# WLBF/flex-gpu-scheduler

Measured on AMD Instinct MI355X. Metric: pods/sec sched throughput + p99 PodGroup gang-admit latency, 1/2/4/8-GPU groups, higher is better.
Workload: dtype int64

## Files before the change

csrc/common/json.cc:

```cpp
#include "common/json.h"

#include <cerrno>
#include <cmath>
#include <cstdio>
#include <cstring>

namespace xsched {

namespace {
const std::string kEmptyString;
const Json::Array kEmptyArray;
const Json::Object kEmptyObject;

class Parser {
 public:
  explicit Parser(std::string_view s) : p_(s.data()), end_(s.data() + s.size()) {}

  Json parse_document() {
    ws();
    Json v = value(0);
    ws();
    if (p_ != end_) fail("trailing characters");
    return v;
  }

  void parse_array_stream(const std::function<void(Json&&)>& fn) {
    ws();
    if (p_ >= end_ || *p_ != '[') fail("expected a JSON array");
    ++p_;
    ws();
    if (p_ < end_ && *p_ == ']') {
      ++p_;
    } else {
      for (;;) {
        ws();
        fn(value(1));
        ws();
        if (p_ < end_ && *p_ == ',') { ++p_; continue; }
        if (p_ < end_ && *p_ == ']') { ++p_; break; }
        fail("expected ',' or ']'");
      }
    }
    ws();
    if (p_ != end_) fail("trailing characters");
  }

 private:
  const char* p_;
  const char* end_;

  [[noreturn]] void fail(const char* what) {
    throw JsonError(std::string("json parse error: ") + what);
  }
  void ws() {
    while (p_ < end_ && (*p_ == ' ' || *p_ == '\n' || *p_ == '\r' || *p_ == '\t')) ++p_;
  }
  bool lit(const char* l, size_t n) {
    if (static_cast<size_t>(end_ - p_) >= n && std::memcmp(p_, l, n) == 0) {
      p_ += n;
      return true;
    }
    return false;
  }

  Json value(int depth) {
    if (depth > 256) fail("nesting too deep");
    if (p_ >= end_) fail("unexpected end");
    switch (*p_) {
      case '{': return object(depth);
      case '[': return array(depth);
      case '"': return Json(string());
      case 't': if (lit("true", 4)) return Json(true); fail("bad literal");
      case 'f': if (lit("false", 5)) return Json(false); fail("bad literal");
      case 'n': if (lit("null", 4)) return Json(); fail("bad literal");
      default: return number();
    }
  }

  Json object(int depth) {
    ++p_;
    Json o = Json::object();
    auto& m = o.members_mut();
    ws();
    if (p_ < end_ && *p_ == '}') { ++p_; return o; }
    for (;;) {
      ws();
      if (p_ >= end_ || *p_ != '"') fail("expected key");
      std::string k = string();
      ws();
      if (p_ >= end_ || *p_ != ':') fail("expected ':'");
      ++p_;
      ws();
      Json v = value(depth + 1);
      bool replaced = false;
      for (auto& kv : m) {
        if (kv.first == k) { kv.second = std::move(v); replaced = true; break; }
      }
      if (!replaced) m.emplace_back(std::move(k), std::move(v));
      ws();
      if (p_ < end_ && *p_ == ',') { ++p_; continue; }
      if (p_ < end_ && *p_ == '}') { ++p_; return o; }
      fail("expected ',' or '}'");
    }
  }

  Json array(int depth) {
    ++p_;
    Json a = Json::array();
    auto& items = a.items_mut();
    ws();
    if (p_ < end_ && *p_ == ']') { ++p_; return a; }
    for (;;) {
      ws();
      items.push_back(value(depth + 1));
      ws();
      if (p_ < end_ && *p_ == ',') { ++p_; continue; }
      if (p_ < end_ && *p_ == ']') { ++p_; return a; }
      fail("expected ',' or ']'");
    }
  }

  static void put_utf8(std::string& out, uint32_t cp) {
    if (cp < 0x80) {
      out.push_back(static_cast<char>(cp));
    } else if (cp < 0x800) {
      out.push_back(static_cast<char>(0xC0 | (cp >> 6)));
      out.push_back(static_cast<char>(0x80 | (cp & 0x3F)));
    } else if (cp < 0x10000) {
      out.push_back(static_cast<char>(0xE0 | (cp >> 12)));
      out.push_back(static_cast<char>(0x80 | ((cp >> 6) & 0x3F)));
      out.push_back(static_cast<char>(0x80 | (cp & 0x3F)));
    } else {
      out.push_back(static_cast<char>(0xF0 | (cp >> 18)));
      out.push_back(static_cast<char>(0x80 | ((cp >> 12) & 0x3F)));
      out.push_back(static_cast<char>(0x80 | ((cp >> 6) & 0x3F)));
      out.push_back(static_cast<char>(0x80 | (cp & 0x3F)));
    }
  }

  uint32_t hex4() {
    if (end_ - p_ < 4) fail("bad \\u escape");
    uint32_t v = 0;
    for (int i = 0; i < 4; ++i) {
      char c = *p_++;
      v <<= 4;
      if (c >= '0' && c <= '9') v |= c - '0';
      else if (c >= 'a' && c <= 'f') v |= c - 'a' + 10;
      else if (c >= 'A' && c <= 'F') v |= c - 'A' + 10;
      else fail("bad hex digit");
    }
    return v;
  }

  std::string string() {
    ++p_;
    std::string out;
    const char* run = p_;
    while (p_ < end_) {
      char c = *p_;
      if (c == '"') {
        out.append(run, p_);
        ++p_;
        return out;
      }
      if (c == '\\') {
        out.append(run, p_);
        ++p_;
        if (p_ >= end_) fail("bad escape");
        char e = *p_++;
        switch (e) {
          case '"': out.push_back('"'); break;
          case '\\': out.push_back('\\'); break;
          case '/': out.push_back('/'); break;
          case 'b': out.push_back('\b'); break;
          case 'f': out.push_back('\f'); break;
          case 'n': out.push_back('\n'); break;
          case 'r': out.push_back('\r'); break;
          case 't': out.push_back('\t'); break;
          case 'u': {
            uint32_t cp = hex4();
            if (cp >= 0xD800 && cp <= 0xDBFF && end_ - p_ >= 6 && p_[0] == '\\' && p_[1] == 'u') {
              p_ += 2;
              uint32_t lo = hex4();
              cp = 0x10000 + ((cp - 0xD800) << 10) + (lo - 0xDC00);
            }
            put_utf8(out, cp);
            break;
          }
          default: fail("bad escape");
        }
        run = p_;
        continue;
      }
      ++p_;
    }
    fail("unterminated string");
  }

  Json number() {
    const char* start = p_;
    bool is_float = false;
    if (p_ < end_ && (*p_ == '-' || *p_ == '+')) ++p_;
    while (p_ < end_) {
      char c = *p_;
      if (c >= '0' && c <= '9') { ++p_; continue; }
      if (c == '.' || c == 'e' || c == 'E' || c == '-' || c == '+') { is_float = true; ++p_; continue; }
      break;
    }
    if (p_ == start) fail("unexpected character");
    std::string tok(start, p_);
    if (!is_float) {
      errno = 0;
      char* e = nullptr;
      long long v = std::strtoll(tok.c_str(), &e, 10);
      if (errno == 0 && e && *e == '\0') return Json(static_cast<int64_t>(v));
    }
    char* e = nullptr;
    double d = std::strtod(tok.c_str(), &e);
    if (!e || *e != '\0') fail("bad number");
    return Json(d);
  }
};

void dump_string(std::string& out, const std::string& s) {
  out.push_back('"');
  for (unsigned char c : s) {
    switch (c) {
      case '"': out += "\\\""; break;
      case '\\': out += "\\\\"; break;
      case '\n': out += "\\n"; break;
      case '\r': out += "\\r"; break;
      case '\t': out += "\\t"; break;
      case '\b': out += "\\b"; break;
      case '\f': out += "\\f"; break;
      default:
        if (c < 0x20) {
          char buf[8];
          std::snprintf(buf, sizeof buf, "\\u%04x", c);
          out += buf;
        } else {
          out.push_back(static_cast<char>(c));
        }
    }
  }
  out.push_back('"');
}
}

const std::string& Json::as_string() const { return t_ == Type::String ? h_.s : kEmptyString; }
const Json::Array& Json::items() const { return t_ == Type::Array ? h_.a : kEmptyArray; }
Json::Array& Json::items_mut() {
  if (t_ != Type::Array) { *this = array(); }
  return h_.a;
}
const Json::Object& Json::members() const { return t_ == Type::Object ? h_.o : kEmptyObject; }
Json::Object& Json::members_mut() {
  if (t_ != Type::Object) { *this = object(); }
  return h_.o;
}

const Json* Json::get(std::string_view key) const {
  if (t_ != Type::Object) return nullptr;
  for (const auto& kv : h_.o)
    if (kv.first == key) return &kv.second;
  return nullptr;
}

Json* Json::get_mut(std::string_view key) {
  if (t_ != Type::Object) return nullptr;
  for (auto& kv : h_.o)
    if (kv.first == key) return &kv.second;
  return nullptr;
}

const Json* Json::path(std::initializer_list<std::string_view> keys) const {
  const Json* cur = this;
  for (auto k : keys) {
    cur = cur->get(k);
    if (!cur) return nullptr;
  }
  return cur;
}

const Json& Json::operator[](std::string_view key) const {
  const Json* v = get(key);
  return v ? *v : json_null();
}

Json& Json::set(std::string_view key, Json v) {
  auto& m = members_mut();
  for (auto& kv : m) {
    if (kv.first == key) {
      kv.second = std::move(v);
      return kv.second;
    }
  }
  m.emplace_back(std::string(key), std::move(v));
  return m.back().second;
}

Json& Json::at_or_create(std::string_view key) {
  auto& m = members_mut();
  for (auto& kv : m)
    if (kv.first == key) {
      if (!kv.second.is_object()) kv.second = object();
      return kv.second;
    }
  m.emplace_back(std::string(key), object());
  return m.back().second;
}

bool Json::erase(std::string_view key) {
  if (t_ != Type::Object) return false;
  for (auto it = h_.o.begin(); it != h_.o.end(); ++it) {
    if (it->first == key) {
      h_.o.erase(it);
      return true;
    }
  }
  return false;
}

void Json::push_back(Json v) { items_mut().push_back(std::move(v)); }

bool Json::operator==(const Json& o) const {
  if (is_number() && o.is_number()) {
    if (t_ == Type::Int && o.t_ == Type::Int) return i_ == o.i_;
    return as_double() == o.as_double();
  }
  if (t_ != o.t_) return false;
  switch (t_) {
    case Type::Null: return true;
    case Type::Bool: return i_ == o.i_;
    case Type::String: return h_.s == o.h_.s;
    case Type::Array: return h_.a == o.h_.a;
    case Type::Object: {
      if (h_.o.size() != o.h_.o.size()) return false;
      for (const auto& kv : h_.o) {
        const Json* other = o.get(kv.first);
        if (!other || !(*other == kv.second)) return false;
      }
      return true;
    }
    default: return false;
  }
}

void Json::dump_to(std::string& out) const {
  switch (t_) {
    case Type::Null: out += "null"; break;
    case Type::Bool: out += i_ ? "true" : "false"; break;
    case Type::Int: out += std::to_string(i_); break;
    case Type::Double: {
      if (!std::isfinite(d_)) { out += "null"; break; }
      char buf[32];
      std::snprintf(buf, sizeof buf, "%.17g", d_);
      out += buf;
      break;
    }
    case Type::String: dump_string(out, h_.s); break;
    case Type::Array: {
      out.push_back('[');
      bool first = true;
      for (const auto& v : h_.a) {
        if (!first) out.push_back(',');
        first = false;
        v.dump_to(out);
      }
      out.push_back(']');
      break;
    }
    case Type::Object: {
      out.push_back('{');
      bool first = true;
      for (const auto& kv : h_.o) {
        if (!first) out.push_back(',');
        first = false;
        dump_string(out, kv.first);
        out.push_back(':');
        kv.second.dump_to(out);
      }
      out.push_back('}');
      break;
    }
  }
}

std::string Json::dump() const {
  std::string out;
  out.reserve(256);
  dump_to(out);
  return out;
}

Json Json::parse(std::string_view text) { return Parser(text).parse_document(); }

void Json::parse_array_stream(std::string_view text, const std::function<void(Json&&)>& fn) {
  Parser(text).parse_array_stream(fn);
}

void Json::merge_patch(const Json& patch) {
  if (!patch.is_object()) {
    *this = patch;
    return;
  }
  if (!is_object()) *this = object();
  for (const auto& kv : patch.h_.o) {
    if (kv.second.is_null()) {
      erase(kv.first);
    } else if (kv.second.is_object()) {
      Json* cur = get_mut(kv.first);
      if (cur && cur->is_object()) {
        cur->merge_patch(kv.second);
      } else {
        Json fresh = object();
        fresh.merge_patch(kv.second);
        set(kv.first, std::move(fresh));
      }
    } else {
      set(kv.first, kv.second);
    }
  }
}

Json Json::diff_merge_patch(const Json& from, const Json& to) {
  if (!from.is_object() || !to.is_object()) return to;
  Json patch = object();
  for (const auto& kv : from.h_.o) {
    if (!to.get(kv.first)) patch.set(kv.first, Json());
  }
  for (const auto& kv : to.h_.o) {
    const Json* old = from.get(kv.first);
    if (!old) {
      patch.set(kv.first, kv.second);
    } else if (!(*old == kv.second)) {
      if (old->is_object() && kv.second.is_object())
        patch.set(kv.first, diff_merge_patch(*old, kv.second));
      else
        patch.set(kv.first, kv.second);
    }
  }
  return patch;
}

namespace {
inline uint64_t mix(uint64_t h, uint64_t v) {
  h ^= v;
  h *= 0xff51afd7ed558ccdULL;
  return h ^ (h >> 33);
}
inline uint64_t fnv(uint64_t h, const void* data, size_t n) {
  const unsigned char* p = static_cast<const unsigned char*>(data);
  h = mix(h, n);
  for (; n >= 8; n -= 8, p += 8) {
    uint64_t w;
    std::memcpy(&w, p, 8);
    h = mix(h, w);
  }
  if (n) {
    uint64_t w = 0;
    std::memcpy(&w, p, n);
    h = mix(h, w);
  }
  return h;
}
}

uint64_t json_hash(const Json& j, uint64_t h, std::string_view skip_key) {
  uint8_t tag = static_cast<uint8_t>(j.type());
  h = fnv(h, &tag, 1);
  switch (j.type()) {
    case Json::Type::Null:
      break;
    case Json::Type::Bool: {
      uint8_t b = j.as_bool() ? 1 : 0;
      h = fnv(h, &b, 1);
      break;
    }
    case Json::Type::Int: {
      int64_t v = j.as_int();
      h = fnv(h, &v, sizeof v);
      break;
    }
    case Json::Type::Double: {
      double v = j.as_double();
      h = fnv(h, &v, sizeof v);
      break;
    }
    case Json::Type::String:
      h = fnv(h, j.as_string().data(), j.as_string().size());
      break;
    case Json::Type::Array:
      for (const auto& x : j.items()) h = json_hash(x, h);
      break;
    case Json::Type::Object:
      for (const auto& [k, v] : j.members()) {
        if (!skip_key.empty() && k == skip_key) continue;
        h = fnv(h, k.data(), k.size());
        h = json_hash(v, h);
      }
      break;
  }
  return h;
}

}
```

csrc/store/store.cc:

```cpp
#include "store/store.h"

#include "common/clock.h"

#include <algorithm>
#include <chrono>
#include <cstdio>
#include <thread>

#include "api/types.h"

namespace xsched {

const char* event_type_name(EventType t) {
  switch (t) {
    case EventType::Added: return "ADDED";
    case EventType::Modified: return "MODIFIED";
    case EventType::Deleted: return "DELETED";
    case EventType::Bookmark: return "BOOKMARK";
  }
  return "UNKNOWN";
}

void Watcher::push(const WatchEvent& ev) {
  {
    std::lock_guard<AdaptiveMutex> g(mu_);
    q_.push_back(ev);
  }
  cv_.notify_one();
}

void Watcher::push_batch(std::vector<WatchEvent> evs) {
  {
    std::lock_guard<AdaptiveMutex> g(mu_);
    for (auto& e : evs) q_.push_back(std::move(e));
  }
  cv_.notify_one();
}

bool Watcher::push_quiet(const WatchEvent& ev) {
  std::lock_guard<AdaptiveMutex> g(mu_);
  q_.push_back(ev);
  return waiters_ > 0;
}

bool Watcher::push_batch_quiet(std::vector<WatchEvent> evs) {
  std::lock_guard<AdaptiveMutex> g(mu_);
  for (auto& e : evs) q_.push_back(std::move(e));
  return waiters_ > 0;
}

std::vector<WatchEvent> Watcher::next(int timeout_ms, size_t max) {
  std::vector<WatchEvent> out;
  std::unique_lock<AdaptiveMutex> lk(mu_);
  if (q_.empty() && !stopped_.load()) {
    ++waiters_;
    if (timeout_ms < 0)
      cv_.wait(lk, [&] { return !q_.empty() || stopped_.load(); });
    else
      cv_.wait_for(lk, std::chrono::milliseconds(timeout_ms), [&] { return !q_.empty() || stopped_.load(); });
    --waiters_;
  }
  size_t n = std::min(max, q_.size());
  out.reserve(n);
  for (size_t i = 0; i < n; ++i) {
    out.push_back(std::move(q_.front()));
    q_.pop_front();
  }
  return out;
}

void Watcher::stop() {
  {
    std::lock_guard<AdaptiveMutex> g(mu_);
    stopped_.store(true);
  }
  cv_.notify_all();
}

size_t Watcher::pending() const {
  std::lock_guard<AdaptiveMutex> g(mu_);
  return q_.size();
}

ObjectStore::~ObjectStore() {
  {
    std::lock_guard<std::mutex> g(reap_mu_);
    reap_stop_ = true;
  }
  reap_cv_.notify_all();
  if (reaper_.joinable()) reaper_.join();
}

void ObjectStore::reap(std::vector<WatchEvent>&& dead) const {
  {
    std::lock_guard<std::mutex> g(reap_mu_);
    if (reap_stop_) return;
    if (!reaper_.joinable()) reaper_ = std::thread([this] { reaper_loop(); });
    if (reap_q_.empty()) {
      reap_q_.swap(dead);
    } else {
      for (auto& e : dead) reap_q_.push_back(std::move(e));
    }
  }
  reap_cv_.notify_one();
}

void ObjectStore::reaper_loop() const {
  name_this_thread("xs-reaper");
  std::unique_lock<std::mutex> lk(reap_mu_);
  for (;;) {
    reap_cv_.wait(lk, [&] { return reap_stop_ || !reap_q_.empty(); });
    std::vector<WatchEvent> batch;
    batch.swap(reap_q_);
    lk.unlock();
    batch.clear();
    lk.lock();
    if (reap_stop_ && reap_q_.empty()) return;
  }
}

ObjectStore::ObjectStore() {
  uid_salt_ = static_cast<uint64_t>(std::chrono::steady_clock::now().time_since_epoch().count());
}

bool ObjectStore::namespaced(const std::string& kind) {
  return !(kind == "nodes" || kind == "priorityclasses" || kind == "noderesourcetopologies" || kind == "namespaces" ||
           kind == "loadwatchermetrics" || kind == "persistentvolumes" || kind == "storageclasses" ||
           kind == "csinodes");
}

void ObjectStore::stamp(Json& obj, int64_t rv) {
  obj.at_or_create("metadata").set("resourceVersion", Json(std::to_string(rv)));
}

void ObjectStore::check_faults(const std::string& verb, const std::string& kind) {
  if (!has_faults_.load(std::memory_order_relaxed)) return;
  int delay = 0;
  bool fail = false;
  {
    std::lock_guard<std::mutex> g(fault_mu_);
    for (auto& r : faults_) {
      if (r.remaining == 0) continue;
      if ((r.verb == "*" || r.verb == verb) && (r.kind == "*" || r.kind == kind)) {
        if (r.remaining > 0) --r.remaining;
        delay += r.delay_us;
        if (r.fail_prob > 0.0 && std::uniform_real_distribution<double>(0, 1)(fault_rng_) < r.fail_prob) fail = true;
      }
    }
  }
  if (delay > 0) std::this_thread::sleep_for(std::chrono::microseconds(delay));
  if (fail) throw StoreError(500, "InternalError", "injected fault: " + verb + " " + kind);
}

void ObjectStore::add_fault(const FaultRule& r) {
  std::lock_guard<std::mutex> g(fault_mu_);
  faults_.push_back(r);
  has_faults_.store(true);
}

void ObjectStore::clear_faults() {
  std::lock_guard<std::mutex> g(fault_mu_);
  faults_.clear();
  has_faults_.store(false);
}

void ObjectStore::emit_locked(EventType t, const std::string& kind, const JsonPtr& obj, const JsonPtr& old, int64_t rv,
                              bool status_only) {
  WatchEvent ev{t, kind, obj, old, rv, status_only};
  if (batch_) {
    batch_->push_back(ev);
  } else {
    const Json& md = (*obj)["metadata"];
    const std::string& ns = md["namespace"].as_string();
    for (auto& w : watchers_)
      if (!w->stopped() && w->wants(kind, ns) && w->push_quiet(ev) &&
          std::find(wake_.begin(), wake_.end(), w) == wake_.end())
        wake_.push_back(w);
  }
  history_.push_back(std::move(ev));
  if (history_.size() > history_cap_) {
    compacted_rv_ = history_.front().rv;
    evicted_.push_back(std::move(history_.front()));
    history_.pop_front();
  }
}

JsonPtr ObjectStore::create_locked(const std::string& kind, Json obj) {
  Json& md = obj.at_or_create("metadata");
  std::string name = md["name"].as_string();
  if (name.empty()) {
    std::string gen = md["generateName"].as_string();
    if (gen.empty()) throw StoreError(422, "Invalid", "metadata.name: Required value");
    char buf[16];
    std::snprintf(buf, sizeof buf, "%05llx", static_cast<unsigned long long>((uid_counter_ * 2654435761u) & 0xfffff));
    name = gen + buf;
    md.set("name", Json(name));
  }
  std::string ns = md["namespace"].as_string();
  if (namespaced(kind) && ns.empty()) {
    ns = "default";
    md.set("namespace", Json(ns));
  }
  auto& km = kinds_[kind];
  std::string key = key_of(namespaced(kind) ? ns : "", name);
  if (km.count(key)) throw StoreError(409, "AlreadyExists", kind + " \"" + name + "\" already exists");
  ++uid_counter_;
  char uid[48];
  uint64_t a = uid_counter_ ^ uid_salt_;
  std::snprintf(uid, sizeof uid, "%08llx-%04llx-4%03llx-8%03llx-%012llx",
                static_cast<unsigned long long>(a & 0xffffffff), static_cast<unsigned long long>((a >> 32) & 0xffff),
                static_cast<unsigned long long>((a >> 48) & 0xfff), static_cast<unsigned long long>(uid_counter_ & 0xfff),
                static_cast<unsigned long long>(uid_counter_));
  if (md["uid"].as_string().empty()) md.set("uid", Json(std::string(uid)));
  if (!md["creationTimestamp"].is_string()) md.set("creationTimestamp", Json(format_rfc3339(wall_now_us())));
  if (kind == "pods") {
    Json& st = obj.at_or_create("status");
    if (!st["phase"].is_string()) st.set("phase", Json("Pending"));
  }
  int64_t rv = rv_.fetch_add(1) + 1;
  stamp(obj, rv);
  auto ptr = std::make_shared<const Json>(std::move(obj));
  km[key] = Entry{ptr};
  emit_locked(EventType::Added, kind, ptr, nullptr, rv);
  if (kind == "events") expire_events_locked(key);
  return ptr;
}

void ObjectStore::set_event_ttl_us(int64_t ttl_us) {
  Guard g(*this);
  event_ttl_us_ = ttl_us;
}

void ObjectStore::expire_events_locked(const std::string& created_key) {
  const int64_t now = wall_now_us();
  event_expiry_.emplace_back(now, created_key);
  auto& km = kinds_["events"];
  while (!event_expiry_.empty() && now - event_expiry_.front().first >= event_ttl_us_) {
    auto it = km.find(event_expiry_.front().second);
    event_expiry_.pop_front();
    if (it == km.end()) continue;
    JsonPtr old = it->second.obj;
    km.erase(it);
    emit_locked(EventType::Deleted, "events", old, old, rv_.fetch_add(1) + 1);
  }
}

JsonPtr ObjectStore::create(const std::string& kind, Json obj) {
  check_faults("create", kind);
  Guard g(*this);
  return create_locked(kind, std::move(obj));
}

std::vector<JsonPtr> ObjectStore::create_many(const std::string& kind, std::vector<Json> objs) {
  check_faults("create", kind);
  std::vector<JsonPtr> out;
  out.reserve(objs.size());
  Guard g(*this);
  std::vector<WatchEvent> batch;
  batch_ = &batch;
  try {
    for (auto& o : objs) out.push_back(create_locked(kind, std::move(o)));
  } catch (...) {
    batch_ = nullptr;
    flush_batch_locked(batch);
    throw;
  }
  batch_ = nullptr;
  flush_batch_locked(batch);
  return out;
}

size_t ObjectStore::create_chunked(const std::string& kind,
                                  const std::function<void(const std::function<void(Json&&)>&)>& produce) {
  auto group_of = [](const Json& o) -> const std::string& {
    return o["metadata"]["labels"]["pod-group.scheduling.sigs.k8s.io"].as_string();
  };
  std::vector<Json> chunk;
  chunk.reserve(2 * kCreateChunk);
  size_t n = 0;
  auto flush = [&] {
    if (chunk.empty()) return;
    n += create_many(kind, std::move(chunk)).size();
    chunk.clear();
  };
  produce([&](Json&& o) {
    if (chunk.size() >= kCreateChunk) {
      const std::string& g = group_of(o);
      if (g.empty() || g != group_of(chunk.back())) flush();
    }
    chunk.push_back(std::move(o));
  });
  flush();
  return n;
}

void ObjectStore::flush_batch_locked(std::vector<WatchEvent>& batch) {
  for (auto& w : watchers_) {
    if (w->stopped()) continue;
    std::vector<WatchEvent> mine;
    mine.reserve(batch.size());
    for (const auto& ev : batch) {
      const std::string& ns = (*ev.obj)["metadata"]["namespace"].as_string();
      if (w->wants(ev.kind, ns)) mine.push_back(ev);
    }
    if (!mine.empty() && w->push_batch_quiet(std::move(mine)) && std::find(wake_.begin(), wake_.end(), w) == wake_.end())
      wake_.push_back(w);
  }
}

JsonPtr ObjectStore::get(const std::string& kind, const std::string& ns, const std::string& name) const {
  Guard g(*this);
  auto kit = kinds_.find(kind);
  if (kit == kinds_.end()) return nullptr;
  auto it = kit->second.find(key_of(namespaced(kind) ? ns : "", name));
  return it == kit->second.end() ? nullptr : it->second.obj;
}

std::vector<JsonPtr> ObjectStore::list(const std::string& kind, const std::string& ns, int64_t* rv_out) const {
  std::vector<JsonPtr> out;
  Guard g(*this);
  if (rv_out) *rv_out = rv_.load();
  auto kit = kinds_.find(kind);
  if (kit == kinds_.end()) return out;
  out.reserve(kit->second.size());
  for (const auto& kv : kit->second) {
    if (!ns.empty() && (*kv.second.obj)["metadata"]["namespace"].as_string() != ns) continue;
    out.push_back(kv.second.obj);
  }
  return out;
}

size_t ObjectStore::count(const std::string& kind) const {
  Guard g(*this);
  auto kit = kinds_.find(kind);
  return kit == kinds_.end() ? 0 : kit->second.size();
}

JsonPtr ObjectStore::update(const std::string& kind, Json obj, bool check_rv) {
  check_faults("update", kind);
  Guard g(*this);
  const Json& md = obj["metadata"];
  std::string ns = namespaced(kind) ? md["namespace"].str_or("default") : "";
  std::string name = md["name"].as_string();
  auto& km = kinds_[kind];
  auto it = km.find(key_of(ns, name));
  if (it == km.end()) throw StoreError(404, "NotFound", kind + " \"" + name + "\" not found");
  const Json& cur_md = (*it->second.obj)["metadata"];
  if (check_rv && md["resourceVersion"].is_string() &&
      md["resourceVersion"].as_string() != cur_md["resourceVersion"].as_string())
    throw StoreError(409, "Conflict",
                     "Operation cannot be fulfilled on " + kind + " \"" + name +
                         "\": the object has been modified; please apply your changes to the latest version and try again");
  Json& nmd = obj.at_or_create("metadata");
  nmd.set("uid", cur_md["uid"]);
  nmd.set("creationTimestamp", cur_md["creationTimestamp"]);
  if (ns.size()) nmd.set("namespace", Json(ns));
  int64_t rv = rv_.fetch_add(1) + 1;
  stamp(obj, rv);
  auto ptr = std::make_shared<const Json>(std::move(obj));
  JsonPtr old = it->second.obj;
  it->second.obj = ptr;
  emit_locked(EventType::Modified, kind, ptr, old, rv);
  return ptr;
}

JsonPtr ObjectStore::update_optimistic(const std::string& kind, const std::string& key, const std::string& name,
                                       const std::function<std::optional<Json>(const Json& cur)>& build,
                                       bool status_only) {
  for (;;) {
    JsonPtr base;
    {
      Guard g(*this);
      auto& km = kinds_[kind];
      auto it = km.find(key);
      if (it == km.end()) throw StoreError(404, "NotFound", kind + " \"" + name + "\" not found");
      base = it->second.obj;
    }
    std::optional<Json> next = build(*base);
    Guard g(*this);
    auto& km = kinds_[kind];
    auto it = km.find(key);
    if (it == km.end()) throw StoreError(404, "NotFound", kind + " \"" + name + "\" not found");
    if (it->second.obj != base) continue;
    if (!next) return base;
    int64_t rv = rv_.fetch_add(1) + 1;
    stamp(*next, rv);
    auto ptr = std::make_shared<const Json>(std::move(*next));
    it->second.obj = ptr;
    emit_locked(EventType::Modified, kind, ptr, base, rv, status_only);
    return ptr;
  }
}

JsonPtr ObjectStore::patch(const std::string& kind, const std::string& ns, const std::string& name,
                           const Json& merge_patch) {
  check_faults("patch", kind);
  bool status_only = merge_patch.is_object() && merge_patch.size() > 0;
  for (const auto& [k, v] : merge_patch.members()) {
    if (k == "status") continue;
    if (k == "metadata" && v.is_object() && v.size() == 1 && v.get("resourceVersion")) continue;
    status_only = false;
  }
  return update_optimistic(kind, key_of(namespaced(kind) ? ns : "", name), name,
                           [&](const Json& cur) -> std::optional<Json> {
    if (const Json* pmd = merge_patch.get("metadata")) {
      const Json& prv = (*pmd)["resourceVersion"];
      if (prv.is_string() && !prv.as_string().empty() && prv.as_string() != cur["metadata"]["resourceVersion"].as_string())
        throw StoreError(409, "Conflict",
                         "Operation cannot be fulfilled on " + kind + " \"" + name +
                             "\": the object has been modified; please apply your changes to the latest version and try again");
    }
    Json obj = cur;
    Json saved_md = obj["metadata"];
    obj.merge_patch(merge_patch);
    Json& md = obj.at_or_create("metadata");
    for (const char* k : {"uid", "creationTimestamp", "name", "namespace"})
      if (const Json* v = saved_md.get(k)) md.set(k, *v);
    if (obj == cur) return std::nullopt;
    return obj;
  }, status_only);
}

JsonPtr ObjectStore::remove(const std::string& kind, const std::string& ns, const std::string& name,
                            int64_t grace_seconds, const std::string& uid_precondition) {
  check_faults("delete", kind);
  Guard g(*this);
  auto& km = kinds_[kind];
  auto it = km.find(key_of(namespaced(kind) ? ns : "", name));
  if (it == km.end()) throw StoreError(404, "NotFound", kind + " \"" + name + "\" not found");
  if (!uid_precondition.empty() && (*it->second.obj)["metadata"]["uid"].as_string() != uid_precondition)
    throw StoreError(409, "Conflict", "Precondition failed: UID in precondition does not match");
  if (kind == "pods" && grace_seconds > 0) {
    Json obj = *it->second.obj;
    Json& md = obj.at_or_create("metadata");
    if (md["deletionTimestamp"].is_string()) return it->second.obj;
    md.set("deletionTimestamp", Json(format_rfc3339(wall_now_us() + grace_seconds * 1000000)));
    md.set("deletionGracePeriodSeconds", Json(grace_seconds));
    int64_t rv = rv_.fetch_add(1) + 1;
    stamp(obj, rv);
    auto ptr = std::make_shared<const Json>(std::move(obj));
    JsonPtr old = it->second.obj;
    it->second.obj = ptr;
    emit_locked(EventType::Modified, kind, ptr, old, rv);
    return ptr;
  }
  JsonPtr old = it->second.obj;
  km.erase(it);
  shrink_locked(km);
  int64_t rv = rv_.fetch_add(1) + 1;
  emit_locked(EventType::Deleted, kind, old, old, rv);
  return old;
}

void ObjectStore::shrink_locked(KindMap& km) {
  if (km.bucket_count() > 4096 && km.size() * 8 < km.bucket_count()) km.rehash(0);
}

size_t ObjectStore::remove_many(const std::string& kind, const std::string& ns,
                                const std::vector<std::string>& names) {
  check_faults("delete", kind);
  Guard g(*this);
  auto& km = kinds_[kind];
  std::vector<WatchEvent> batch;
  batch_ = &batch;
  size_t n = 0;
  for (const auto& name : names) {
    auto it = km.find(key_of(namespaced(kind) ? ns : "", name));
    if (it == km.end()) continue;
    JsonPtr old = it->second.obj;
    km.erase(it);
    int64_t rv = rv_.fetch_add(1) + 1;
    emit_locked(EventType::Deleted, kind, old, old, rv);
    ++n;
  }
  shrink_locked(km);
  batch_ = nullptr;
  flush_batch_locked(batch);
  return n;
}

size_t ObjectStore::delete_all(const std::string& kind, const std::string& ns) {
  Guard g(*this);
  auto kit = kinds_.find(kind);
  if (kit == kinds_.end()) return 0;
  size_t n = 0;
  std::vector<WatchEvent> batch;
  batch_ = &batch;
  struct Flush {
    ObjectStore* s;
    std::vector<WatchEvent>* b;
    ~Flush() {
      s->batch_ = nullptr;
      s->flush_batch_locked(*b);
    }
  } flush{this, &batch};
  for (auto it = kit->second.begin(); it != kit->second.end();) {
    if (!ns.empty() && (*it->second.obj)["metadata"]["namespace"].as_string() != ns) {
      ++it;
      continue;
    }
    JsonPtr old = it->second.obj;
    it = kit->second.erase(it);
    int64_t rv = rv_.fetch_add(1) + 1;
    emit_locked(EventType::Deleted, kind, old, old, rv);
    ++n;
    if (batch.size() >= kCreateChunk) {
      flush_batch_locked(batch);
      batch.clear();
    }
  }
  return n;
}

JsonPtr ObjectStore::bind(const std::string& ns, const std::string& name, const std::string& uid,
                          const std::string& node, const Json& annotations) {
  check_faults("bind", "pods");
  const std::string now = format_rfc3339(wall_now_us());
  return update_optimistic("pods", key_of(ns, name), name, [&](const Json& cur) -> std::optional<Json> {
    if (!uid.empty() && cur["metadata"]["uid"].as_string() != uid)
      throw StoreError(409, "Conflict", "Precondition failed: UID in precondition does not match");
    if (!cur["spec"]["nodeName"].as_string().empty())
      throw StoreError(409, "Conflict",
                       "pod " + name + " is already assigned to node \"" + cur["spec"]["nodeName"].as_string() + "\"");
    if (cur["metadata"]["deletionTimestamp"].is_string())
      throw StoreError(409, "Conflict", "pod " + name + " is being deleted, cannot be assigned to a host");
    Json obj = cur;
    obj.at_or_create("spec").set("nodeName", Json(node));
    if (annotations.is_object() && annotations.size()) {
      Json& ann = obj.at_or_create("metadata").at_or_create("annotations");
      for (const auto& kv : annotations.members()) ann.set(kv.first, kv.second);
    }
    Json& st = obj.at_or_create("status");
    Json cond = Json::object();
    cond.set("type", Json("PodScheduled"));
    cond.set("status", Json("True"));
    cond.set("lastTransitionTime", Json(now));
    Json conds = Json::array();
    for (const auto& c : st["conditions"].items())
      if (c["type"].as_string() != "PodScheduled") conds.push_back(c);
    conds.push_back(std::move(cond));
    st.set("conditions", std::move(conds));
    return obj;
  });
}

WatcherPtr ObjectStore::watch(const std::set<std::string>& kinds, const std::string& ns, int64_t since_rv) {
  auto w = std::make_shared<Watcher>(kinds, ns);
  Guard g(*this);
  if (since_rv > 0) {
    if (since_rv < compacted_rv_)
      throw StoreError(410, "Expired", "too old resource version: " + std::to_string(since_rv));
    for (const auto& ev : history_) {
      if (ev.rv <= since_rv) continue;
      const std::string& ens = (*ev.obj)["metadata"]["namespace"].as_string();
      if (w->wants(ev.kind, ens)) w->push(ev);
    }
  }
  watchers_.push_back(w);
  return w;
}

void ObjectStore::unwatch(const WatcherPtr& w) {
  w->stop();
  Guard g(*this);
  for (auto it = watchers_.begin(); it != watchers_.end(); ++it) {
    if (*it == w) {
      watchers_.erase(it);
      break;
    }
  }
}

}
```

csrc/store/store.h:

```cpp
#pragma once

#include "common/adaptive_mutex.h"

#include <atomic>
#include <condition_variable>
#include <cstdint>
#include <deque>
#include <functional>
#include <map>
#include <memory>
#include <mutex>
#include <optional>
#include <random>
#include <set>
#include <string>
#include <thread>
#include <unordered_map>
#include <vector>

#include "common/json.h"

namespace xsched {

class StoreError : public std::runtime_error {
 public:
  StoreError(int code, const std::string& reason, const std::string& msg)
      : std::runtime_error(msg), code_(code), reason_(reason) {}
  int code() const { return code_; }
  const std::string& reason() const { return reason_; }

 private:
  int code_;
  std::string reason_;
};

enum class EventType : uint8_t { Added, Modified, Deleted, Bookmark };
const char* event_type_name(EventType t);

struct WatchEvent {
  EventType type;
  std::string kind;
  JsonPtr obj;
  JsonPtr old;
  int64_t rv = 0;
  bool status_only = false;
};

class Watcher {
 public:
  explicit Watcher(std::set<std::string> kinds, std::string ns) : kinds_(std::move(kinds)), ns_(std::move(ns)) {}
  std::vector<WatchEvent> next(int timeout_ms, size_t max = 4096);
  void stop();
  bool stopped() const { return stopped_.load(); }
  size_t pending() const;
  bool wants(const std::string& kind, const std::string& ns) const {
    return (kinds_.empty() || kinds_.count(kind)) && (ns_.empty() || ns.empty() || ns == ns_);
  }
  void push(const WatchEvent& ev);
  void push_batch(std::vector<WatchEvent> evs);
  bool push_quiet(const WatchEvent& ev);
  bool push_batch_quiet(std::vector<WatchEvent> evs);
  void notify() { cv_.notify_one(); }

 private:
  std::set<std::string> kinds_;
  std::string ns_;
  mutable AdaptiveMutex mu_;
  std::condition_variable_any cv_;
  std::deque<WatchEvent> q_;
  int waiters_ = 0;
  std::atomic<bool> stopped_{false};
};
using WatcherPtr = std::shared_ptr<Watcher>;

struct FaultRule {
  std::string verb;
  std::string kind;
  double fail_prob = 0.0;
  int delay_us = 0;
  int remaining = -1;
};

class ObjectStore {
 public:
  ObjectStore();
  ~ObjectStore();

  JsonPtr create(const std::string& kind, Json obj);
  JsonPtr get(const std::string& kind, const std::string& ns, const std::string& name) const;
  std::vector<JsonPtr> list(const std::string& kind, const std::string& ns, int64_t* rv_out = nullptr) const;
  JsonPtr update(const std::string& kind, Json obj, bool check_rv = true);
  JsonPtr patch(const std::string& kind, const std::string& ns, const std::string& name, const Json& merge_patch);
  JsonPtr remove(const std::string& kind, const std::string& ns, const std::string& name, int64_t grace_seconds = 0,
                 const std::string& uid_precondition = "");
  JsonPtr bind(const std::string& ns, const std::string& name, const std::string& uid, const std::string& node,
               const Json& annotations);

  WatcherPtr watch(const std::set<std::string>& kinds, const std::string& ns = "", int64_t since_rv = 0);
  void unwatch(const WatcherPtr& w);

  int64_t resource_version() const { return rv_.load(); }
  size_t count(const std::string& kind) const;

  void add_fault(const FaultRule& r);
  void clear_faults();

  void set_event_ttl_us(int64_t ttl_us);

  std::vector<JsonPtr> create_many(const std::string& kind, std::vector<Json> objs);
  static constexpr size_t kCreateChunk = 64;
  size_t create_chunked(const std::string& kind,
                        const std::function<void(const std::function<void(Json&&)>&)>& produce);
  size_t delete_all(const std::string& kind, const std::string& ns = "");
  size_t remove_many(const std::string& kind, const std::string& ns, const std::vector<std::string>& names);

  static std::string key_of(const std::string& ns, const std::string& name) { return ns.empty() ? name : ns + "/" + name; }
  static bool namespaced(const std::string& kind);

 private:
  struct Entry {
    JsonPtr obj;
  };
  using KindMap = std::unordered_map<std::string, Entry>;

  void check_faults(const std::string& verb, const std::string& kind);
  void expire_events_locked(const std::string& created_key);
  void emit_locked(EventType t, const std::string& kind, const JsonPtr& obj, const JsonPtr& old, int64_t rv,
                   bool status_only = false);
  JsonPtr create_locked(const std::string& kind, Json obj);
  void flush_batch_locked(std::vector<WatchEvent>& batch);
  static void stamp(Json& obj, int64_t rv);
  JsonPtr update_optimistic(const std::string& kind, const std::string& key, const std::string& name,
                            const std::function<std::optional<Json>(const Json& cur)>& build, bool status_only = false);
  std::vector<WatchEvent>* batch_ = nullptr;

  mutable AdaptiveMutex mu_;
  class Guard {
   public:
    explicit Guard(const ObjectStore& s) : s_(s) { s_.mu_.lock(); }
    ~Guard() {
      std::vector<WatchEvent> dead;
      if (!s_.evicted_.empty()) dead.swap(s_.evicted_);
      std::vector<WatcherPtr> wake;
      if (!s_.wake_.empty()) wake.swap(s_.wake_);
      s_.mu_.unlock();
      for (const auto& w : wake) w->notify();
      if (!dead.empty()) s_.reap(std::move(dead));
    }
    Guard(const Guard&) = delete;
    Guard& operator=(const Guard&) = delete;

   private:
    const ObjectStore& s_;
  };
  mutable std::vector<WatchEvent> evicted_;
  mutable std::vector<WatcherPtr> wake_;
  void reap(std::vector<WatchEvent>&& dead) const;
  void reaper_loop() const;
  mutable std::mutex reap_mu_;
  mutable std::condition_variable reap_cv_;
  mutable std::vector<WatchEvent> reap_q_;
  mutable std::thread reaper_;
  mutable bool reap_stop_ = false;
  void shrink_locked(KindMap& km);
  std::unordered_map<std::string, KindMap> kinds_;
  std::atomic<int64_t> rv_{0};
  std::vector<WatcherPtr> watchers_;
  std::deque<WatchEvent> history_;
  size_t history_cap_ = 50000;
  int64_t event_ttl_us_ = 3600LL * 1000000;
  std::deque<std::pair<int64_t, std::string>> event_expiry_;
  int64_t compacted_rv_ = 0;
  uint64_t uid_counter_ = 0;
  uint64_t uid_salt_;

  std::mutex fault_mu_;
  std::vector<FaultRule> faults_;
  std::atomic<bool> has_faults_{false};
  std::mt19937_64 fault_rng_{12345};
};

}
```

flex_gpu_scheduler_amd/build_ext.py:

```python
from __future__ import annotations

import argparse
import concurrent.futures as cf
import os
import shutil
import subprocess
import sys
import sysconfig
from pathlib import Path

ROOT = Path(__file__).resolve().parent.parent
CSRC = ROOT / "csrc"
PKG = ROOT / "flex_gpu_scheduler_amd"
BUILD = ROOT / "build"
HIP_ARCH = os.environ.get("PYTORCH_ROCM_ARCH", "gfx950")
ROCM = Path(os.environ.get("ROCM_PATH", "/opt/rocm"))

CORE_DIRS = ["common", "api", "store", "framework", "scheduler", "plugins", "rest", "apiserver"]
LINK_LIBS = ["-lssl", "-lcrypto"]
CXXFLAGS = ["-std=c++20", "-O3", "-fPIC", "-Wall", "-Wno-unused-variable", "-Wno-unused-parameter",
            "-Wno-sign-compare", "-fvisibility=hidden", "-pthread",
            *os.environ.get("XSCHED_CXXFLAGS_EXTRA", "").split()]


def _ext_suffix() -> str:
    return sysconfig.get_config_var("EXT_SUFFIX") or ".so"


def core_sources() -> list[Path]:
    out = []
    for d in CORE_DIRS:
        out.extend(sorted((CSRC / d).glob("*.cc")))
    return out


def _headers_mtime() -> float:
    hs = list(CSRC.rglob("*.h"))
    return max((h.stat().st_mtime for h in hs), default=0.0)


def _jobs() -> int:
    env = os.environ.get("MAX_JOBS")
    if env and env.isdigit():
        return max(1, int(env))
    return max(1, min(16, os.cpu_count() or 4))


def _compile(cmd: list[str], src: Path) -> None:
    r = subprocess.run(cmd, capture_output=True, text=True)
    if r.returncode != 0:
        raise RuntimeError(f"compile failed for {src}:\n{' '.join(cmd)}\n{r.stderr[-8000:]}")


def build_objects(srcs: list[Path], objdir: Path, extra: list[str], includes: list[str]) -> list[Path]:
    objdir.mkdir(parents=True, exist_ok=True)
    hmt = _headers_mtime()
    todo = []
    objs = []
    for s in srcs:
        o = objdir / (s.relative_to(CSRC).as_posix().replace("/", "__") + ".o")
        objs.append(o)
        if o.exists() and o.stat().st_mtime >= max(s.stat().st_mtime, hmt):
            continue
        cmd = ["g++", *CXXFLAGS, *extra, *[f"-I{i}" for i in includes], "-c", str(s), "-o", str(o)]
        todo.append((cmd, s))
    if todo:
        with cf.ThreadPoolExecutor(_jobs()) as ex:
            futs = [ex.submit(_compile, c, s) for c, s in todo]
            for f in futs:
                f.result()
    return objs


def build_core(verbose: bool = True) -> Path:
    import pybind11

    py_inc = sysconfig.get_paths()["include"]
    includes = [str(CSRC), pybind11.get_include(), py_inc, str(ROCM / "include")]
    srcs = core_sources() + sorted((CSRC / "telemetry").glob("*.cc")) + [CSRC / "python" / "bindings.cc"]
    objs = build_objects(srcs, BUILD / "core", [], includes)
    out = PKG / f"_xsched{_ext_suffix()}"
    newest = max(o.stat().st_mtime for o in objs)
    if not out.exists() or out.stat().st_mtime < newest:
        cmd = ["g++", "-shared", "-pthread", *[str(o) for o in objs], *LINK_LIBS, "-o", str(out)]
        r = subprocess.run(cmd, capture_output=True, text=True)
        if r.returncode != 0:
            raise RuntimeError(f"link failed:\n{r.stderr[-8000:]}")
        if verbose:
            print(f"[build_ext] linked {out.relative_to(ROOT)}")
    return out


def build_core_debuginfo(verbose: bool = True) -> Path:
    import pybind11

    py_inc = sysconfig.get_paths()["include"]
    includes = [str(CSRC), pybind11.get_include(), py_inc, str(ROCM / "include")]
    srcs = core_sources() + sorted((CSRC / "telemetry").glob("*.cc")) + [CSRC / "python" / "bindings.cc"]
    objs = build_objects(srcs, BUILD / "core_g", ["-g1", "-gz"], includes)
    out = ROOT / "dbg" / f"_xsched{_ext_suffix()}"
    out.parent.mkdir(exist_ok=True)
    cmd = ["g++", "-shared", "-pthread", *[str(o) for o in objs], *LINK_LIBS, "-o", str(out)]
    r = subprocess.run(cmd, capture_output=True, text=True)
    if r.returncode != 0:
        raise RuntimeError(f"link failed:\n{r.stderr[-8000:]}")
    if verbose:
        print(f"[build_ext] linked {out.relative_to(ROOT)}")
    return out


def build_hip(verbose: bool = True) -> Path | None:
    hipcc = shutil.which("hipcc") or str(ROCM / "bin" / "hipcc")
    if not Path(hipcc).exists():
        raise RuntimeError("hipcc not found; the HIP probes require ROCm")
    srcs = sorted((CSRC / "hip").glob("*.hip"))
    if not srcs:
        return None
    out = PKG / "ops" / "_hipprobe.so"
    newest = max([s.stat().st_mtime for s in srcs] + [_headers_mtime()])
    if out.exists() and out.stat().st_mtime >= newest:
        return out
    cmd = [hipcc, f"--offload-arch={HIP_ARCH}", "-O3", "-std=c++17", "-fPIC", "-shared",
           f"-I{CSRC}", *[str(s) for s in srcs], "-o", str(out)]
    r = subprocess.run(cmd, capture_output=True, text=True)
    if r.returncode != 0:
        raise RuntimeError(f"hipcc failed:\n{' '.join(cmd)}\n{r.stderr[-8000:]}")
    if verbose:
        print(f"[build_ext] built {out.relative_to(ROOT)} for {HIP_ARCH}")
    return out


def build_stream_sweep(verbose: bool = True) -> Path:
    hipcc = shutil.which("hipcc") or str(ROCM / "bin" / "hipcc")
    src = CSRC / "tools" / "stream_sweep.hip"
    out = PKG / "ops" / "stream_sweep"
    if out.exists() and out.stat().st_mtime >= src.stat().st_mtime:
        return out
    cmd = [hipcc, f"--offload-arch={HIP_ARCH}", "-O3", "-std=c++17", str(src), "-o", str(out)]
    r = subprocess.run(cmd, capture_output=True, text=True)
    if r.returncode != 0:
        raise RuntimeError(f"hipcc failed:\n{' '.join(cmd)}\n{r.stderr[-8000:]}")
    if verbose:
        print(f"[build_ext] built {out.relative_to(ROOT)} for {HIP_ARCH}")
    return out


def build_tsan(verbose: bool = True) -> Path:
    includes = [str(CSRC)]
    extra = ["-fsanitize=thread", "-g", "-O1", "-include", str(CSRC / "tools" / "tsan_compat.h")]
    objs = build_objects(core_sources() + [CSRC / "tools" / "stress_main.cc"], BUILD / "tsan", extra, includes)
    out = BUILD / "xsched_stress_tsan"
    cmd = ["g++", "-fsanitize=thread", "-pthread", *[str(o) for o in objs], *LINK_LIBS, "-o", str(out)]
    r = subprocess.run(cmd, capture_output=True, text=True)
    if r.returncode != 0:
        raise RuntimeError(f"tsan link failed:\n{r.stderr[-8000:]}")
    if verbose:
        print(f"[build_ext] built {out.relative_to(ROOT)}")
    return out


def build_asan(verbose: bool = True) -> Path:
    includes = [str(CSRC)]
    flags = ["-fsanitize=address,undefined", "-fno-omit-frame-pointer"]
    objs = build_objects(core_sources() + [CSRC / "tools" / "stress_main.cc"], BUILD / "asan", [*flags, "-g", "-O1"],
                         includes)
    out = BUILD / "xsched_stress_asan"
    cmd = ["g++", *flags, "-pthread", *[str(o) for o in objs], *LINK_LIBS, "-o", str(out)]
    r = subprocess.run(cmd, capture_output=True, text=True)
    if r.returncode != 0:
        raise RuntimeError(f"asan link failed:\n{r.stderr[-8000:]}")
    if verbose:
        print(f"[build_ext] built {out.relative_to(ROOT)}")
    return out


def build_prof(verbose: bool = True, gprof: bool = True, debuginfo: bool = False) -> Path:
    includes = [str(CSRC)]
    extra = ["-pg", "-g", "-O2", "-fno-omit-frame-pointer", "-fno-inline-functions-called-once"] if gprof else []
    if debuginfo and not gprof:
        extra = ["-g"]
    sub = "prof" if gprof else ("stress_g" if debuginfo else "stress")
    objs = build_objects(core_sources() + [CSRC / "tools" / "stress_main.cc"], BUILD / sub, extra, includes)
    out = BUILD / ("xsched_stress_prof" if gprof else ("xsched_stress_g" if debuginfo else "xsched_stress"))
    cmd = ["g++", *(["-pg"] if gprof else []), "-pthread", *[str(o) for o in objs], *LINK_LIBS, "-o", str(out)]
    r = subprocess.run(cmd, capture_output=True, text=True)
    if r.returncode != 0:
        raise RuntimeError(f"prof link failed:\n{r.stderr[-8000:]}")
    if verbose:
        print(f"[build_ext] built {out.relative_to(ROOT)}")
    return out


def build_stress_count(verbose: bool = True, debuginfo: bool = False) -> Path:
    includes = [str(CSRC)]
    extra = ["-g1", "-fno-omit-frame-pointer"] if debuginfo else []
    srcs = core_sources() + [CSRC / "tools" / "stress_main.cc", CSRC / "tools" / "alloc_count.cc"]
    objs = build_objects(srcs, BUILD / ("stress_count_g" if debuginfo else "core"), extra, includes)
    out = BUILD / ("xsched_stress_count_g" if debuginfo else "xsched_stress_count")
    newest = max(o.stat().st_mtime for o in objs)
    if out.exists() and out.stat().st_mtime >= newest:
        return out
    cmd = ["g++", "-pthread", *[str(o) for o in objs], *LINK_LIBS, "-ldl", "-o", str(out)]
    r = subprocess.run(cmd, capture_output=True, text=True)
    if r.returncode != 0:
        raise RuntimeError(f"stress-count link failed:\n{r.stderr[-8000:]}")
    if verbose:
        print(f"[build_ext] built {out.relative_to(ROOT)}")
    return out


def build_tests(verbose: bool = True) -> Path:
    includes = [str(CSRC)]
    objs = build_objects(core_sources() + [CSRC / "tests" / "native_tests.cc"], BUILD / "core", [], includes)
    out = BUILD / "xsched_native_tests"
    newest = max(o.stat().st_mtime for o in objs)
    if out.exists() and out.stat().st_mtime >= newest:
        return out
    cmd = ["g++", "-pthread", *[str(o) for o in objs], *LINK_LIBS, "-o", str(out)]
    r = subprocess.run(cmd, capture_output=True, text=True)
    if r.returncode != 0:
        raise RuntimeError(f"native tests link failed:\n{r.stderr[-8000:]}")
    if verbose:
        print(f"[build_ext] built {out.relative_to(ROOT)}")
    return out


def build_gang_tests(verbose: bool = True, tsan: bool = False) -> Path:
    includes = [str(CSRC)]
    extra = ["-fsanitize=thread", "-g", "-O1", "-include", str(CSRC / "tools" / "tsan_compat.h")] if tsan else []
    objs = build_objects(core_sources() + [CSRC / "tests" / "gang_tests.cc"], BUILD / ("tsan" if tsan else "core"),
                         extra, includes)
    out = BUILD / ("xsched_gang_tests_tsan" if tsan else "xsched_gang_tests")
    newest = max(o.stat().st_mtime for o in objs)
    if out.exists() and out.stat().st_mtime >= newest:
        return out
    cmd = ["g++", *(["-fsanitize=thread"] if tsan else []), "-pthread", *[str(o) for o in objs], *LINK_LIBS,
           "-o", str(out)]
    r = subprocess.run(cmd, capture_output=True, text=True)
    if r.returncode != 0:
        raise RuntimeError(f"gang tests link failed:\n{r.stderr[-8000:]}")
    if verbose:
        print(f"[build_ext] built {out.relative_to(ROOT)}")
    return out


def main(argv: list[str] | None = None) -> int:
    ap = argparse.ArgumentParser()
    ap.add_argument("--core", action="store_true")
    ap.add_argument("--hip", action="store_true")
    ap.add_argument("--tsan", action="store_true")
    ap.add_argument("--asan", action="store_true")
    ap.add_argument("--prof", action="store_true")
    ap.add_argument("--stress", action="store_true")
    ap.add_argument("--stress-g", action="store_true", help="stress driver with -g (sample_report --lines)")
    ap.add_argument("--stress-count", action="store_true",
                    help="stress driver with the counting operator new/delete (allocations per thread)")
    ap.add_argument("--stress-count-g", action="store_true", help="the same with line tables (call stacks)")
    ap.add_argument("--tests", action="store_true")
    ap.add_argument("--core-g", action="store_true", help="the extension with -g into dbg/ (sampling runs)")
    ap.add_argument("--gang-tests", action="store_true", help="native tests of the lister's gang entries")
    ap.add_argument("--gang-tests-tsan", action="store_true", help="the same under ThreadSanitizer (host only)")
    a = ap.parse_args(argv)
    if a.gang_tests or a.gang_tests_tsan:
        build_gang_tests(tsan=a.gang_tests_tsan)
        return 0
    if a.core_g:
        build_core_debuginfo()
        return 0
    if a.tests:
        build_tests()
        return 0
    if a.stress_count or a.stress_count_g:
        build_stress_count(debuginfo=a.stress_count_g)
        return 0
    if a.prof or a.stress or a.stress_g:
        build_prof(gprof=a.prof, debuginfo=a.stress_g)
        return 0
    everything = not (a.core or a.hip or a.tsan or a.asan)
    if a.core or everything:
        build_core()
    if a.hip or everything:
        build_hip()
    if a.tsan:
        build_tsan()
    if a.asan:
        build_asan()
    return 0


if __name__ == "__main__":
    sys.exit(main())
```

Baseline: 140,500.

## Reduce allocations in JSON parse, object creation and batched watch fan-out

The JSON parser now collects object members and array items in per-depth scratch vectors and moves them into an exactly reserved container when the closing bracket is reached, to avoid repeated vector regrowth. The store's create path pre-reserves metadata and top-level members, swaps snprintf for a hand-written hex uid formatter that runs only when a uid is missing, and caches the kind comparisons. Batch flushing reserves the batch and, when exactly one watcher wants every event, moves the whole batch to it instead of copying per watcher. It also adds build targets for unit tests. The changes add code complexity and an extra move pass per container in the parser.

```diff
diff --git a/csrc/common/json.cc b/csrc/common/json.cc
--- a/csrc/common/json.cc
+++ b/csrc/common/json.cc
@@ -77,12 +77,17 @@
     }
   }
 
+  std::vector<Json::Object> members_at_;
+  std::vector<Json::Array> items_at_;
+
   Json object(int depth) {
     ++p_;
     Json o = Json::object();
-    auto& m = o.members_mut();
     ws();
     if (p_ < end_ && *p_ == '}') { ++p_; return o; }
+    const size_t d = static_cast<size_t>(depth);
+    if (members_at_.size() <= d) members_at_.resize(d + 1);
+    members_at_[d].clear();
     for (;;) {
       ws();
       if (p_ >= end_ || *p_ != '"') fail("expected key");
@@ -92,6 +97,7 @@
       ++p_;
       ws();
       Json v = value(depth + 1);
+      auto& m = members_at_[d];
       bool replaced = false;
       for (auto& kv : m) {
         if (kv.first == k) { kv.second = std::move(v); replaced = true; break; }
@@ -99,7 +105,14 @@
       if (!replaced) m.emplace_back(std::move(k), std::move(v));
       ws();
       if (p_ < end_ && *p_ == ',') { ++p_; continue; }
-      if (p_ < end_ && *p_ == '}') { ++p_; return o; }
+      if (p_ < end_ && *p_ == '}') {
+        ++p_;
+        auto& out = o.members_mut();
+        out.reserve(m.size());
+        for (auto& kv : m) out.push_back(std::move(kv));
+        m.clear();
+        return o;
+      }
       fail("expected ',' or '}'");
     }
   }
@@ -107,15 +120,26 @@
   Json array(int depth) {
     ++p_;
     Json a = Json::array();
-    auto& items = a.items_mut();
     ws();
     if (p_ < end_ && *p_ == ']') { ++p_; return a; }
+    const size_t d = static_cast<size_t>(depth);
+    if (items_at_.size() <= d) items_at_.resize(d + 1);
+    items_at_[d].clear();
     for (;;) {
       ws();
-      items.push_back(value(depth + 1));
+      Json v = value(depth + 1);
+      auto& items = items_at_[d];
+      items.push_back(std::move(v));
       ws();
       if (p_ < end_ && *p_ == ',') { ++p_; continue; }
-      if (p_ < end_ && *p_ == ']') { ++p_; return a; }
+      if (p_ < end_ && *p_ == ']') {
+        ++p_;
+        auto& out = a.items_mut();
+        out.reserve(items.size());
+        for (auto& x : items) out.push_back(std::move(x));
+        items.clear();
+        return a;
+      }
       fail("expected ',' or ']'");
     }
   }
diff --git a/csrc/store/store.cc b/csrc/store/store.cc
--- a/csrc/store/store.cc
+++ b/csrc/store/store.cc
@@ -185,8 +185,50 @@
   }
 }
 
+void ObjectStore::format_uid(char out[48], uint64_t counter, uint64_t salt) {
+  static const char kHex[] = "0123456789abcdef";
+  const uint64_t a = counter ^ salt;
+  char* p = out;
+  auto hex = [&](uint64_t v, int width) {
+    int n = 1;
+    for (uint64_t t = v >> 4; t; t >>= 4) ++n;
+    if (n < width) n = width;
+    for (int i = n - 1; i >= 0; --i, v >>= 4) p[i] = kHex[v & 0xf];
+    p += n;
+  };
+  hex(a & 0xffffffff, 8);
+  *p++ = '-';
+  hex((a >> 32) & 0xffff, 4);
+  *p++ = '-';
+  *p++ = '4';
+  hex((a >> 48) & 0xfff, 3);
+  *p++ = '-';
+  *p++ = '8';
+  hex(counter & 0xfff, 3);
+  *p++ = '-';
+  hex(counter, 12);
+  *p = '\0';
+}
+
 JsonPtr ObjectStore::create_locked(const std::string& kind, Json obj) {
+  using namespace std::string_view_literals;
+  const bool is_pod = kind == "pods"sv;
+  const bool wants_ns = namespaced(kind);
+  if (obj.is_object()) {
+    size_t add = (obj.get("metadata") ? 0 : 1) + (is_pod && !obj.get("status") ? 1 : 0);
+    if (add) obj.members_mut().reserve(obj.size() + add);
+  }
   Json& md = obj.at_or_create("metadata");
+  {
+    size_t add = wants_ns ? 5 : 4;
+    for (const auto& kv : md.members()) {
+      const std::string_view k = kv.first;
+      if (k == "name"sv || (wants_ns && k == "namespace"sv) || k == "uid"sv || k == "creationTimestamp"sv ||
+          k == "resourceVersion"sv)
+        --add;
+    }
+    if (add) md.members_mut().reserve(md.size() + add);
+  }
   std::string name = md["name"].as_string();
   if (name.empty()) {
     std::string gen = md["generateName"].as_string();
@@ -197,23 +239,21 @@
     md.set("name", Json(name));
   }
   std::string ns = md["namespace"].as_string();
-  if (namespaced(kind) && ns.empty()) {
+  if (wants_ns && ns.empty()) {
     ns = "default";
     md.set("namespace", Json(ns));
   }
   auto& km = kinds_[kind];
-  std::string key = key_of(namespaced(kind) ? ns : "", name);
+  std::string key = key_of(wants_ns ? ns : "", name);
   if (km.count(key)) throw StoreError(409, "AlreadyExists", kind + " \"" + name + "\" already exists");
   ++uid_counter_;
-  char uid[48];
-  uint64_t a = uid_counter_ ^ uid_salt_;
-  std::snprintf(uid, sizeof uid, "%08llx-%04llx-4%03llx-8%03llx-%012llx",
-                static_cast<unsigned long long>(a & 0xffffffff), static_cast<unsigned long long>((a >> 32) & 0xffff),
-                static_cast<unsigned long long>((a >> 48) & 0xfff), static_cast<unsigned long long>(uid_counter_ & 0xfff),
-                static_cast<unsigned long long>(uid_counter_));
-  if (md["uid"].as_string().empty()) md.set("uid", Json(std::string(uid)));
+  if (md["uid"].as_string().empty()) {
+    char uid[48];
+    format_uid(uid, uid_counter_, uid_salt_);
+    md.set("uid", Json(std::string(uid)));
+  }
   if (!md["creationTimestamp"].is_string()) md.set("creationTimestamp", Json(format_rfc3339(wall_now_us())));
-  if (kind == "pods") {
+  if (is_pod) {
     Json& st = obj.at_or_create("status");
     if (!st["phase"].is_string()) st.set("phase", Json("Pending"));
   }
@@ -222,7 +262,7 @@
   auto ptr = std::make_shared<const Json>(std::move(obj));
   km[key] = Entry{ptr};
   emit_locked(EventType::Added, kind, ptr, nullptr, rv);
-  if (kind == "events") expire_events_locked(key);
+  if (kind == "events"sv) expire_events_locked(key);
   return ptr;
 }
 
@@ -257,6 +297,7 @@
   out.reserve(objs.size());
   Guard g(*this);
   std::vector<WatchEvent> batch;
+  batch.reserve(objs.size());
   batch_ = &batch;
   try {
     for (auto& o : objs) out.push_back(create_locked(kind, std::move(o)));
@@ -295,14 +336,39 @@
 }
 
 void ObjectStore::flush_batch_locked(std::vector<WatchEvent>& batch) {
+  if (batch.empty()) return;
+  auto wants = [](const Watcher& w, const WatchEvent& ev) {
+    return w.wants(ev.kind, (*ev.obj)["metadata"]["namespace"].as_string());
+  };
+  const WatcherPtr* sole = nullptr;
+  for (const auto& w : watchers_) {
+    if (w->stopped()) continue;
+    if (sole) {
+      if (std::any_of(batch.begin(), batch.end(), [&](const WatchEvent& ev) { return wants(*w, ev); })) {
+        sole = nullptr;
+        break;
+      }
+      continue;
+    }
+    size_t n = 0;
+    for (const auto& ev : batch) n += wants(*w, ev) ? 1 : 0;
+    if (n == 0) continue;
+    if (n < batch.size()) break;
+    sole = &w;
+  }
+  if (sole) {
+    const WatcherPtr& w = *sole;
+    if (w->push_batch_quiet(std::move(batch)) && std::find(wake_.begin(), wake_.end(), w) == wake_.end())
+      wake_.push_back(w);
+    batch.clear();
+    return;
+  }
   for (auto& w : watchers_) {
     if (w->stopped()) continue;
     std::vector<WatchEvent> mine;
     mine.reserve(batch.size());
-    for (const auto& ev : batch) {
-      const std::string& ns = (*ev.obj)["metadata"]["namespace"].as_string();
-      if (w->wants(ev.kind, ns)) mine.push_back(ev);
-    }
+    for (const auto& ev : batch)
+      if (wants(*w, ev)) mine.push_back(ev);
     if (!mine.empty() && w->push_batch_quiet(std::move(mine)) && std::find(wake_.begin(), wake_.end(), w) == wake_.end())
       wake_.push_back(w);
   }
diff --git a/csrc/store/store.h b/csrc/store/store.h
--- a/csrc/store/store.h
+++ b/csrc/store/store.h
@@ -116,6 +116,7 @@
 
   static std::string key_of(const std::string& ns, const std::string& name) { return ns.empty() ? name : ns + "/" + name; }
   static bool namespaced(const std::string& kind);
+  static void format_uid(char out[48], uint64_t counter, uint64_t salt);
 
  private:
   struct Entry {
diff --git a/flex_gpu_scheduler_amd/build_ext.py b/flex_gpu_scheduler_amd/build_ext.py
--- a/flex_gpu_scheduler_amd/build_ext.py
+++ b/flex_gpu_scheduler_amd/build_ext.py
@@ -244,6 +244,30 @@
     return out
 
 
+UNIT_TESTS = ("json_tests", "store_tests")
+
+
+def build_unit_tests(name: str, verbose: bool = True, asan: bool = False) -> Path:
+    if name not in UNIT_TESTS:
+        raise ValueError(f"unknown unit test program {name!r}; one of {UNIT_TESTS}")
+    includes = [str(CSRC)]
+    flags = ["-fsanitize=address,undefined", "-fno-omit-frame-pointer"] if asan else []
+    extra = [*flags, "-g", "-O1"] if asan else []
+    objs = build_objects(core_sources() + [CSRC / "tests" / f"{name}.cc"], BUILD / ("asan" if asan else "core"),
+                         extra, includes)
+    out = BUILD / (f"xsched_{name}_asan" if asan else f"xsched_{name}")
+    newest = max(o.stat().st_mtime for o in objs)
+    if out.exists() and out.stat().st_mtime >= newest:
+        return out
+    cmd = ["g++", *flags, "-pthread", *[str(o) for o in objs], *LINK_LIBS, "-o", str(out)]
+    r = subprocess.run(cmd, capture_output=True, text=True)
+    if r.returncode != 0:
+        raise RuntimeError(f"{name} link failed:\n{r.stderr[-8000:]}")
+    if verbose:
+        print(f"[build_ext] built {out.relative_to(ROOT)}")
+    return out
+
+
 def main(argv: list[str] | None = None) -> int:
     ap = argparse.ArgumentParser()
     ap.add_argument("--core", action="store_true")
@@ -260,7 +284,12 @@
     ap.add_argument("--core-g", action="store_true", help="the extension with -g into dbg/ (sampling runs)")
     ap.add_argument("--gang-tests", action="store_true", help="native tests of the lister's gang entries")
     ap.add_argument("--gang-tests-tsan", action="store_true", help="the same under ThreadSanitizer (host only)")
+    ap.add_argument("--unit-tests", choices=UNIT_TESTS, help="one native test program of csrc/tests")
+    ap.add_argument("--unit-tests-asan", choices=UNIT_TESTS, help="the same under ASan + UBSan (host only)")
     a = ap.parse_args(argv)
+    if a.unit_tests or a.unit_tests_asan:
+        build_unit_tests(a.unit_tests or a.unit_tests_asan, asan=bool(a.unit_tests_asan))
+        return 0
     if a.gang_tests or a.gang_tests_tsan:
         build_gang_tests(tsan=a.gang_tests_tsan)
         return 0
```

Measured after the change: 139,900. Within noise of the previous version (-0.5%).
